# yjpark1/multiagent_rl

Measured on AMD Instinct MI355X. Metric: env-steps/sec, simple_spread N=6 x B envs, 1/2/4/8 MI355X, higher is better.
Workload: dtype f32

## Files before the change

multiagent_rl_amd/csrc/pw_kernels_spread_quad.hpp:

```cpp
#pragma once

#include "pw_kernels_spread.hpp"

namespace {

__device__ __forceinline__ void quad_pair_of(const int q, int &i, int &j)
{
    i = q < 5 ? 0 : q < 9 ? 1 : q < 12 ? 2 : q < 14 ? 3 : 4;
    j = q - (i == 0 ? 0 : i == 1 ? 5 : i == 2 ? 9 : i == 3 ? 12 : 14) + i + 1;
}

__device__ __forceinline__ void quad_act_fetch(const int32_t *row, const uint32_t lane_off, const uint32_t lds_slot, const uint32_t slot_read)
{
    unsigned keep;
    asm volatile("s_mov_b32 %0, m0\n\ts_mov_b32 m0, %3\n\ts_nop 0\n\tglobal_load_lds_dword %1, %2\n\ts_mov_b32 m0, %0"
                 : "=&s"(keep) : "v"(lane_off), "s"(row), "s"(lds_slot), "v"(slot_read) : "memory");
}

__device__ __forceinline__ float2 quad_action_force(const int ai, const float sens, const float fscale)
{
    float ux = 0.0f + ((ai == 1 ? 1.0f : 0.0f) - (ai == 2 ? 1.0f : 0.0f));
    float uy = 0.0f + ((ai == 3 ? 1.0f : 0.0f) - (ai == 4 ? 1.0f : 0.0f));
    ux *= sens; uy *= sens;
    if (fscale != 1.0f) { ux = fscale * ux; uy = fscale * uy; }
    return make_float2(ux + 0.0f, uy + 0.0f);
}

template <bool K1>
__device__ __forceinline__ void quad_pair_force(const float2 qi, const float2 qj, const uint32_t near_lo, const uint32_t near_span,
                                                const float dist_min, const float k, const float cf, float &Fx, float &Fy)
{
    const float dx = qi.x - qj.x, dy = qi.y - qj.y;
    const float d2 = dx * dx + dy * dy;
    const f32x2 a = {cf * dx, cf * dy};
    const bool near = __float_as_uint(d2) - near_lo >= near_span;
    const bool uni = (k >= 9.094947017729282e-13f) & (k <= 1099511627776.0f) & (cf >= 9.5367431640625e-07f) & (cf <= 128.0f);
    const bool c1 = (__float_as_uint(d2) - 0x12800000u) < (0x6C800000u - 0x12800000u);
    const bool c2 = fminf(fabsf(a.x), fabsf(a.y)) >= 8.673617379884035e-19f;
    const bool fast = near & c1 & c2 & uni;
    const bool any_cold = __builtin_amdgcn_ballot_w64(near & !fast) != 0;
    Fx = 0.0f; Fy = 0.0f;
    if (fast) {
        const float dist = sqrt_rn_core(d2);
        const float y0 = __builtin_amdgcn_rcpf(dist);
        __builtin_amdgcn_sched_barrier(0);
        const float yd = __builtin_fmaf(__builtin_fmaf(-dist, y0, 1.0f), y0, y0);
        const f32x2 Q = div_chain2(a, dist, yd);
        const float xarg = K1 ? div_chain1(-(dist - dist_min), k, div_refined_rcp(k))
                              : div_chain(-(dist - dist_min), k, div_refined_rcp(k));
        const float pen = softplus_branchless(xarg) * k;
        const f32x2 F = Q * f32x2{pen, pen};
        Fx = F.x;
        Fy = F.y;
    }
    if (__builtin_expect(any_cold, 0)) {
        if (near & !fast) collision_force_pair<true, K1>(qi.x, qi.y, qj.x, qj.y, dist_min, k, cf, Fx, Fy);
    }
}

template <bool COLL>
__device__ __forceinline__ void quad_coll_tests(const float2 mine, const float2 (&q6)[6], const float coll_thr2, int &cnt, uint32_t &cmask)
{
    cnt = 0; cmask = 0;
#if defined(PW_EXPERIMENTS) && defined(PW_EXP_NO_COLL_TESTS)
    cnt = 1;
#else
#pragma unroll
    for (int j = 0; j < 6; ++j) {
        const float2 q = q6[j];
        const float dx = q.x - mine.x, dy = q.y - mine.y;
        const float d2 = dx * dx + dy * dy;
        cnt += d2 < coll_thr2 ? 1 : 0;
        if (COLL) cmask |= d2 < coll_thr2 ? 1u << j : 0u;
    }
#endif
}

#ifndef PW_QUAD_BARRIER
#define PW_QUAD_BARRIER(t) duo_barrier()
#endif
#ifndef PW_QUAD_ACT_AHEAD
#define PW_QUAD_ACT_AHEAD 4
#endif
#ifndef PW_QUAD_PAD_P
#define PW_QUAD_PAD_P()
#endif
#ifndef PW_QUAD_PAD_OB
#define PW_QUAD_PAD_OB()
#endif
constexpr int kQuadActAhead = PW_QUAD_ACT_AHEAD;
constexpr int kQuadN = 6, kQuadL = 6, kQuadEPP = 4, kQuadEPW = 8;
struct SpreadQuadLds { float4 *s_ring; float2 *s_ftab, *s_lmB, *s_utab, *s_u; float *s_min, *s_rew; int32_t *s_act; uint32_t bytes; };
__host__ __device__ inline SpreadQuadLds spread_quad_lds(unsigned char *raw = nullptr)
{
    LdsCursor c{reinterpret_cast<float *>(raw)}; SpreadQuadLds o;
    o.s_ring = c.take<float4>(4 * kWave);
    o.s_ftab = c.take<float2>(2 * kQuadEPP * kQuadN * kQuadN);
    o.s_min = c.take<float>(kWave); o.s_rew = c.take<float>(kWave);
    o.s_lmB = c.take<float2>(kQuadEPW * kQuadL); o.s_act = c.take<int32_t>(2 * kQuadActAhead * kWave);
    o.s_u = reinterpret_cast<float2 *>(o.s_act + kQuadActAhead * kWave);
    o.s_utab = c.take<float2>(2 * 8);
    o.bytes = 4 * c.at; return o;
}
template <bool UNIT_MASS, bool COLL = false, bool K1 = false>
__global__ void __launch_bounds__(4 * kWave) pw_spread_quad_kernel(const StreamParams A, const int T)
{
    constexpr int N = kQuadN, L = kQuadL, D = 16, P2 = 15, EPP = kQuadEPP, EPW = kQuadEPW;
    extern __shared__ __attribute__((aligned(16))) unsigned char smem_raw[];
    const SpreadQuadLds Y = spread_quad_lds(smem_raw);

    const int wave = __builtin_amdgcn_readfirstlane((((int)threadIdx.x >> 6) + 2 * (((int)blockIdx.x >> 8) & 1)) & 3);
    const int lane = (int)threadIdx.x & 63;
    const int env0 = (int)blockIdx.x * EPW;
    const int envs_here = A.B - env0 < EPW ? A.B - env0 : EPW;
    const size_t BN = (size_t)A.B * N;

    const bool resets = A.auto_reset && A.max_episode_len > 0;
    int offs_all = A.ep_step[env0 + (lane < envs_here ? lane : 0)];
    auto next_reset_step = [&](int t_from) -> int {
        if (!resets) return 0x7fffffff;
        int rem = A.max_episode_len - 1 - (t_from + offs_all);
        rem = rem < 0 ? 0 : rem;
        int m = 0x7fffffff;
        for (int e = 0; e < envs_here; ++e) {
            const int r = __builtin_amdgcn_readlane(rem, e);
            m = r < m ? r : m;
        }
        return t_from + m;
    };
    int t_reset = next_reset_step(0);
    auto reset_step_update = [&](int t) {
        if (t + 1 + offs_all >= A.max_episode_len) offs_all = -(t + 1);
        t_reset = next_reset_step(t + 1);
    };
    int cur = 0;

    if (wave < 2) {
        __builtin_amdgcn_s_setprio(3);
        const int e0 = wave * EPP;
        const int nv = envs_here - e0 < 0 ? 0 : envs_here - e0 < EPP ? envs_here - e0 : EPP;
        if (nv == 0) {
            for (int t = 0; t < T; ++t) PW_QUAD_BARRIER(t);
            return;
        }
        const int la = lane < nv * N ? lane : 0;
        const int e4 = la / N, a = la - e4 * N;
        const int me = (e0 + e4) * N + a;
        const int env = env0 + e0 + e4;
        const uint32_t g = (uint32_t)env * (uint32_t)N + (uint32_t)a;
        const uint64_t env_id = A.env_id_base + (uint64_t)env;
        const int lp = lane < nv * P2 ? lane : 0;
        const int pe = lp / P2, pq = lp - pe * P2;
        int pi, pj;
        quad_pair_of(pq, pi, pj);
        const int ri = (e0 + pe) * N + pi, rj = (e0 + pe) * N + pj;
        float2 *ftab = Y.s_ftab + wave * (EPP * N * N);
        float2 *f_ij = ftab + (pe * N + pi) * N + (pj - 1), *f_ji = ftab + (pe * N + pj) * N + pi;
        const float2 *row = ftab + (e4 * N + a) * N;

        float px = A.pos_x[g], py = A.pos_y[g], vx = A.vel_x[g], vy = A.vel_y[g];
        int ep_off = A.ep_step[env];
        uint32_t ep_count = A.ep_count[env];
        Y.s_ring[me] = make_float4(px, py, vx, vy);
        float2 *u_w = Y.s_u + me;
        {
            const int32_t a0 = A.act[g], a1 = A.act[(T > 1 ? BN : (size_t)0) + g];
            u_w[0] = quad_action_force(a0, A.sens, A.fscale);
            u_w[kQuadEPW * N] = quad_action_force(a1, A.sens, A.fscale);
        }
        int u_at = 0;
        const float k = A.contact_margin, cf = A.contact_force, dt = A.dt, damp = A.damp, mass = A.mass;
        const uint32_t near_lo = __float_as_uint(A.near_thr2), near_span = 0x7F800000u - near_lo;
        float2 qi = *reinterpret_cast<const float2 *>(Y.s_ring + ri);
        float2 qj = *reinterpret_cast<const float2 *>(Y.s_ring + rj);
        PW_STAMP_DECL;
        for (int t = 0; t < T; ++t) {
            PW_STAMP_START;
            const float2 u0 = u_w[u_at];
            u_at = kQuadEPW * N - u_at;
            const bool two_slots = t == t_reset;
            float Fx, Fy;
            quad_pair_force<K1>(qi, qj, near_lo, near_span, A.dist_min, k, cf, Fx, Fy);
            *f_ij = make_float2(Fx, Fy);
            *f_ji = make_float2(-Fx, -Fy);
            PW_STAMP(0);
            float fx = u0.x, fy = u0.y;
            asm volatile("" ::: "memory");
#pragma unroll
            for (int j = 0; j < N - 1; ++j) {
                const float2 F = row[j];
                fx = F.x + fx;
                fy = F.y + fy;
            }
            vx = vx * damp; vy = vy * damp;
            vx = vx + div_mass<UNIT_MASS>(fx, mass) * dt;
            vy = vy + div_mass<UNIT_MASS>(fy, mass) * dt;
            px = px + vx * dt;
            py = py + vy * dt;
            int nxt = (cur + 1) & 3;
            Y.s_ring[nxt * kWave + me] = make_float4(px, py, vx, vy);
            if (__builtin_expect(two_slots, 0)) {
                if (t + 1 + ep_off >= A.max_episode_len) {
                    ep_count += 1;
                    ep_off = -(t + 1);
                    pw_reset_xy(A.seed, env_id, ep_count, (uint32_t)a, -1.0f, 1.0f, &px, &py);
                    vx = 0.f; vy = 0.f;
                }
                reset_step_update(t);
                nxt = (nxt + 1) & 3;
                Y.s_ring[nxt * kWave + me] = make_float4(px, py, vx, vy);
            }
            cur = nxt;
            asm volatile("" ::: "memory");
            qi = *reinterpret_cast<const float2 *>(Y.s_ring + cur * kWave + ri);
            qj = *reinterpret_cast<const float2 *>(Y.s_ring + cur * kWave + rj);
            PW_STAMP(1);
            PW_QUAD_PAD_P();
            PW_QUAD_BARRIER(t);
            PW_STAMP(2);
        }
#ifdef PW_STAMPS
        if (blockIdx.x == 0 && wave == 0 && lane == 0)
            for (int i_ = 0; i_ < 4; ++i_) g_pw_stamps[i_] = st_acc[i_];
#endif
        A.pos_x[g] = px; A.pos_y[g] = py;
        A.vel_x[g] = vx; A.vel_y[g] = vy;
        A.ep_step[env] = T + ep_off;
        A.ep_count[env] = ep_count;
        return;
    }

    int e_local = lane / N;
    int a = lane - e_local * N;
    if (e_local >= envs_here) { e_local = 0; a = 0; }
    const int env = env0 + e_local;
    const int base = e_local * N, me = base + a;
    const uint32_t g = (uint32_t)env * (uint32_t)N + (uint32_t)a;
    const uint64_t env_id = A.env_id_base + (uint64_t)env;
    int ep_off = A.ep_step[env];
    uint32_t ep_count = A.ep_count[env];
    float olx = A.lm_x[(size_t)env * L + a], oly = A.lm_y[(size_t)env * L + a];

    if (wave == 2) {
        float own_p = 0.0f;
        int cnt_p = 0;
        const int *cnt_w = reinterpret_cast<const int *>(Y.s_min) + lane;
        const int cnt_span = (int)(Y.s_rew - Y.s_min);
        int cnt_at = 0;
        int pre_last = 0;
        float2 q6[N];
        auto a_reads = [&](const int nxt) __attribute__((always_inline)) {
            const float4 *slot = Y.s_ring + nxt * kWave + base;
#pragma unroll
            for (int j = 0; j < N; ++j) q6[j] = *reinterpret_cast<const float2 *>(slot + j);
            pre_last = nxt;
        };
        float best, e0;
        auto a_dist = [&]() __attribute__((always_inline)) {
            float e2[N];
#pragma unroll
            for (int j = 0; j < N; ++j) {
                const float2 q = q6[j];
                const float ex = q.x - olx, ey = q.y - oly;
                e2[j] = ex * ex + ey * ey;
            }
            best = __builtin_fminf(__builtin_fminf(__builtin_fminf(e2[0], e2[1]), __builtin_fminf(e2[2], e2[3])),
                                   __builtin_fminf(e2[4], e2[5]));
            e0 = e2[0];
        };
        auto a_sqrt = [&]() __attribute__((always_inline)) -> float {
            const float b = e0 != e0 ? e0 : best;
            return sqrtf(b);
        };
        auto a_clock = [&](const int t, int nxt) __attribute__((always_inline)) {
            if (__builtin_expect(t == t_reset, 0)) {
                if (t + 1 + ep_off >= A.max_episode_len) {
                    ep_count += 1;
                    ep_off = -(t + 1);
                    pw_reset_xy(A.seed, env_id, ep_count, (uint32_t)(N + a), -1.0f, 1.0f, &olx, &oly);
                }
                reset_step_update(t);
                nxt = (nxt + 1) & 3;
            }
            cur = nxt;
        };
        float sh_own[L], sh_r[N], r;
        auto b_shfl_own = [&]() __attribute__((always_inline)) {
#pragma unroll
            for (int l = 0; l < L; ++l) sh_own[l] = __shfl(own_p, base + l, kWave);
        };
        auto b_reward = [&]() __attribute__((always_inline)) {
            r = 0.0f;
#pragma unroll
            for (int l = 0; l < L; ++l) r -= sh_own[l];
#pragma unroll
            for (int k2 = 0; k2 < N; ++k2) r -= k2 < cnt_p ? 1.0f : 0.0f;
#pragma unroll
            for (int i = 0; i < N; ++i) sh_r[i] = __shfl(r, base + i, kWave);
        };
        float *rew_t = A.rew, *rsh_t = A.rew_shared;
        auto b_store = [&]() __attribute__((always_inline)) {
            float acc = 0.0f;
#pragma unroll
            for (int i = 0; i < N; ++i) acc += sh_r[i];
            nt_store(rew_t + g, r);
            nt_store(rsh_t + env, acc);
            rew_t += BN; rsh_t += A.B;
        };
        PW_STAMP_DECL;
        {
            PW_STAMP_START;
            PW_QUAD_BARRIER(0);
            PW_STAMP(0);
            const int nxt = (cur + 1) & 3;
            a_reads(nxt);
            a_dist();
            own_p = a_sqrt();
            a_clock(0, nxt);
            PW_STAMP(1);
        }
        for (int t = 1; t < T; ++t) {
            PW_STAMP_START;
            PW_QUAD_BARRIER(t);
            PW_STAMP(0);
            const int nxt = (cur + 1) & 3;
            cnt_p = cnt_w[cnt_at];
            cnt_at = cnt_span - cnt_at;
            a_reads(nxt);
            b_shfl_own();
            a_dist();
            b_reward();
            const float own = a_sqrt();
            b_store();
            own_p = own;
            a_clock(t, nxt);
            PW_STAMP(1);
        }
        {
            const float4 *slot = Y.s_ring + pre_last * kWave + base;
            const float2 mine = *reinterpret_cast<const float2 *>(slot + a);
#pragma unroll
            for (int j = 0; j < N; ++j) q6[j] = *reinterpret_cast<const float2 *>(slot + j);
            uint32_t cmask;
            quad_coll_tests<false>(mine, q6, A.coll_thr2, cnt_p, cmask);
        }
        b_shfl_own();
        b_reward();
        b_store();
#ifdef PW_STAMPS
        if (blockIdx.x == 0 && lane == 0)
            for (int i_ = 0; i_ < 2; ++i_) g_pw_stamps[4 + i_] = st_acc[i_];
#endif
        return;
    }

    const int rows_here = envs_here * N;
    const int cgrp = lane & 3;
    const bool col0 = cgrp == 0;
    int row_u[3];
    uint32_t off_u[3];
#pragma unroll
    for (int u = 0; u < 3; ++u) {
        const int r = (lane >> 2) + 16 * u;
        const bool ok = r < rows_here;
        row_u[u] = ok ? r : 0;
        off_u[u] = (uint32_t)(ok ? lane + 64 * u : cgrp) * 16u;
    }
    float4 lm_u[3];
    auto load_landmarks = [&]() {
#pragma unroll
        for (int u = 0; u < 3; ++u)
            lm_u[u] = *reinterpret_cast<const float4 *>(Y.s_lmB + (row_u[u] / N) * L + (cgrp > 0 ? 2 * cgrp - 2 : 0));
    };
    Y.s_lmB[me] = make_float2(olx, oly);
    constexpr int kStepStores = 5 + (COLL ? 1 : 0);
    constexpr int kActBehind = kQuadActAhead * kStepStores + kQuadActAhead - 1;
    constexpr int kActWait = kActBehind < 63 ? kActBehind : 63;
    const unsigned char *act_row = reinterpret_cast<const unsigned char *>(A.act) + (size_t)(T > 2 ? 2 : T > 0 ? T - 1 : 0) * (BN * sizeof(int32_t));
    const size_t act_stride = BN * sizeof(int32_t);
    const uint32_t act_off = g * (uint32_t)sizeof(int32_t);
    const unsigned char *act_ring = reinterpret_cast<const unsigned char *>(Y.s_act + lane);
    uint32_t act_lds = __builtin_amdgcn_readfirstlane((uint32_t)reinterpret_cast<uintptr_t>(Y.s_act));
    asm volatile("" : "+s"(act_lds));
    constexpr uint32_t kSlotBytes = kWave * sizeof(int32_t), kRingMask = kQuadActAhead * kSlotBytes - 1;
    auto fetch_act = [&](int s, uint32_t slot_at, uint32_t slot_read) {
        quad_act_fetch(reinterpret_cast<const int32_t *>(act_row), act_off, act_lds + slot_at, slot_read);
        act_row += s + 1 < T ? act_stride : (size_t)0;
    };
    asm volatile("" :: "v"(ep_off), "v"(ep_count), "v"(offs_all), "v"(olx), "v"(oly), "s"(t_reset));
    for (int s0 = 2; s0 < 2 + kQuadActAhead; ++s0) fetch_act(s0, ((uint32_t)s0 * kSlotBytes) & kRingMask, 0u);
    if (lane < 6) Y.s_utab[lane] = quad_action_force(lane, A.sens, A.fscale);
    float2 *u_w = Y.s_u + me;
    int u_at = 0;
    uint32_t act_slot = (2 * kSlotBytes) & kRingMask;
    wave_lds_sync();
    load_landmarks();
    act_fetch_drain();
    unsigned char *obs_t = reinterpret_cast<unsigned char *>(A.obs + ((size_t)env0 * N) * D);
    uint8_t *done_t = A.done, *term_t = A.terminal;
    const size_t obs_stride = BN * D * sizeof(float);
    const bool has_len = A.max_episode_len > 0;
    int t_term = has_len ? A.max_episode_len - 1 - ep_off : 0x7fffffff;
    int *cnt_w = reinterpret_cast<int *>(Y.s_min) + lane;
    const int cnt_span = (int)(Y.s_rew - Y.s_min);
    int cnt_at = 0;
    uint64_t *coll_t = A.coll;
    PW_STAMP_DECL;
    for (int t = 0; t < T; ++t) {
        PW_STAMP_START;
        nt_store(done_t + g, (uint8_t)0);
        PW_QUAD_BARRIER(t);
        PW_STAMP(0);
        asm volatile("s_waitcnt vmcnt(%0)" :: "n"(kActWait) : "memory");
        const uint32_t ai = *reinterpret_cast<const uint32_t *>(act_ring + act_slot);
        int nxt = (cur + 1) & 3;
        float2 cmine, cq6[N];
        {
            const float4 *pre = Y.s_ring + nxt * kWave + base;
            cmine = *reinterpret_cast<const float2 *>(pre + a);
#pragma unroll
            for (int j = 0; j < N; ++j) cq6[j] = *reinterpret_cast<const float2 *>(pre + j);
        }
        fetch_act(t + 2 + kQuadActAhead, act_slot, ai);
        act_slot = (act_slot + kSlotBytes) & kRingMask;
        const float2 u2 = Y.s_utab[ai < 5u ? ai : 5u];
        nt_store(term_t + env, (uint8_t)(t >= t_term ? 1 : 0));
        if (t == t_reset) {
            const bool rst = t >= t_term;
            if (rst) {
                if (A.final_obs) {
                    const float4 st = Y.s_ring[nxt * kWave + me];
                    stream_write_obs<L>(A.final_obs + ((size_t)t * BN + g) * D, L, Y.s_lmB + base, st.x, st.y, st.z, st.w);
                }
                ep_count += 1;
                ep_off = -(t + 1);
                t_term = A.max_episode_len - 1 - ep_off;
                pw_reset_xy(A.seed, env_id, ep_count, (uint32_t)(N + a), -1.0f, 1.0f, &olx, &oly);
            }
            reset_step_update(t);
            wave_lds_sync();
            if (rst) Y.s_lmB[me] = make_float2(olx, oly);
            wave_lds_sync();
            load_landmarks();
            nxt = (nxt + 1) & 3;
        }
        cur = nxt;
        const float4 *slot = Y.s_ring + nxt * kWave;
        float4 st[3];
#pragma unroll
        for (int u = 0; u < 3; ++u) st[u] = slot[row_u[u]];
        {
            int cnt;
            uint32_t cmask;
            quad_coll_tests<COLL>(cmine, cq6, A.coll_thr2, cnt, cmask);
            cnt_w[cnt_at] = cnt;
            cnt_at = cnt_span - cnt_at;
            u_w[u_at] = u2;
            u_at = kQuadEPW * N - u_at;
            if (COLL) {
                nt_store(coll_t + g, (uint64_t)cmask);
                coll_t += BN;
            }
        }
        asm volatile("" :: "v"(st[0].x), "v"(st[0].y), "v"(st[0].z), "v"(st[0].w), "v"(st[1].x), "v"(st[1].y), "v"(st[1].z),
                           "v"(st[1].w), "v"(st[2].x), "v"(st[2].y), "v"(st[2].z), "v"(st[2].w));
#pragma unroll
        for (int u = 0; u < 3; ++u) {
            const float4 d = make_float4(lm_u[u].x - st[u].x, lm_u[u].y - st[u].y, lm_u[u].z - st[u].x, lm_u[u].w - st[u].y);
            const float4 o = make_float4(col0 ? st[u].z : d.x, col0 ? st[u].w : d.y, col0 ? st[u].x : d.z, col0 ? st[u].y : d.w);
            nt_store(reinterpret_cast<float4 *>(obs_t + off_u[u]), o);
        }
        obs_t += obs_stride; done_t += BN; term_t += A.B;
        PW_QUAD_PAD_OB();
        PW_STAMP(1);
    }
#ifdef PW_STAMPS
    if (blockIdx.x == 0 && lane == 0)
        for (int i_ = 0; i_ < 2; ++i_) g_pw_stamps[6 + i_] = st_acc[i_];
#endif
    A.lm_x[(size_t)env * L + a] = olx;
    A.lm_y[(size_t)env * L + a] = oly;
    act_fetch_drain();
}

}
```

multiagent_rl_amd/env.py:

```python
import ctypes as C

import numpy as np
import torch

from . import _lib
from ._lib import PwConfig, PwStateLayout, PwStepIO, check


class Discrete(object):

    def __init__(self, n):
        self.n = n
        self.shape = ()

    def sample(self):
        return int(np.random.randint(self.n))

    def __repr__(self):
        return 'Discrete(%d)' % self.n


class MultiDiscrete(object):

    def __init__(self, array_of_param_array):
        self.low = np.array([x[0] for x in array_of_param_array])
        self.high = np.array([x[1] for x in array_of_param_array])
        self.num_discrete_space = self.low.shape[0]
        self.shape = (self.num_discrete_space,)

    def sample(self):
        return [int(np.random.randint(lo, hi + 1)) for lo, hi in zip(self.low, self.high)]

    def __repr__(self):
        return 'MultiDiscrete' + str(self.num_discrete_space)


class Box(object):
    def __init__(self, shape, dtype=np.float32):
        self.shape = tuple(shape)
        self.dtype = dtype
        self.low, self.high_ = -np.inf, np.inf

    def __repr__(self):
        return 'Box%s' % (self.shape,)


def _ptr(t):
    return None if t is None else C.c_void_p(t.data_ptr())


def make_config(scenario_name, num_envs, num_agents=None, num_landmarks=None, num_adversaries=None,
                num_good=None, local_observation=True, max_episode_len=25, auto_reset=False,
                force_discrete_action=True, seed=12345678, env_id_base=0, action_force_uses_accel=False,
                **constants):
    lib = _lib.load()
    if scenario_name not in _lib.SCENARIOS:
        raise ValueError('unsupported scenario: %r (supported: %s)' % (scenario_name, sorted(_lib.SCENARIOS)))
    scen = _lib.SCENARIOS[scenario_name]
    if scen in (_lib.PW_SIMPLE_REFERENCE, _lib.PW_SIMPLE_SPEAKER_LISTENER):
        adv, n = 0, 2
    elif scen == _lib.PW_SIMPLE_TAG:
        adv = 3 if num_adversaries is None else int(num_adversaries)
        if num_good is None:
            num_good = 1 if num_agents is None else int(num_agents) - adv
        n = adv + int(num_good)
    else:
        adv = 0
        n = 3 if num_agents is None else int(num_agents)
    cfg = PwConfig()
    check(lib.pw_config_default(C.byref(cfg), scen, int(num_envs), n,
                                -1 if num_landmarks is None else int(num_landmarks), adv))
    cfg.obs_mode = _lib.PW_OBS_LOCAL if local_observation else _lib.PW_OBS_FULL
    cfg.max_episode_len = int(max_episode_len)
    cfg.auto_reset = int(bool(auto_reset))
    cfg.force_discrete_action = int(bool(force_discrete_action))
    cfg.action_force_uses_accel = int(bool(action_force_uses_accel))
    cfg.seed = int(seed) & 0xFFFFFFFFFFFFFFFF
    cfg.env_id_base = int(env_id_base)
    for k, v in constants.items():
        if k not in ('dt', 'damping', 'contact_force', 'contact_margin', 'default_sensitivity', 'mass',
                     'landmark_size'):
            raise TypeError('unknown world constant %r' % k)
        setattr(cfg, k, float(v))
    return cfg


class BatchedParticleEnv(object):

    def __init__(self, scenario_name='simple_spread', num_envs=1, device=None, config=None, want_coll=False,
                 dispatch=None, **kw):
        self.lib = _lib.load()
        if not torch.cuda.is_available():
            raise _lib.PworldError('BatchedParticleEnv needs a GPU: libpworld has no CPU fallback')
        self.device = torch.device('cuda', torch.cuda.current_device()) if device is None else torch.device(device)
        self.cfg = config if config is not None else make_config(scenario_name, num_envs, **kw)
        self.scenario_name = scenario_name
        h = C.c_void_p()
        check(self.lib.pw_create(C.byref(self.cfg), C.byref(h)))
        self._h = h
        if dispatch:
            self.set_dispatch(**dispatch)
        self.num_envs, self.n = self.cfg.num_envs, self.cfg.num_agents
        self.num_landmarks = self.cfg.num_landmarks
        self.obs_dim = self.lib.pw_obs_dim(h)
        self.want_coll = want_coll
        self.observation_space = [Box((self.obs_dim,)) for _ in range(self.n)]
        self.speaker_listener = self.cfg.scenario == _lib.PW_SIMPLE_SPEAKER_LISTENER
        self.dim_c = {_lib.PW_SIMPLE_REFERENCE: _lib.PW_DIM_C,
                      _lib.PW_SIMPLE_SPEAKER_LISTENER: _lib.PW_SL_DIM_C}.get(self.cfg.scenario, 0)
        if self.speaker_listener:
            if self.cfg.obs_mode != _lib.PW_OBS_LOCAL:
                raise NotImplementedError('simple_speaker_listener: only the observation the reference patches in '
                                          '(experiments/scenarios.py:45-64, local_observation=True) is built; '
                                          "upstream's has a different length per agent")
            self.action_space = [Discrete(self.dim_c), Discrete(5)]
            self.act_width = 5
        else:
            self.action_space = [MultiDiscrete([[0, 4], [0, self.dim_c - 1]]) if self.dim_c else Discrete(5)
                                 for _ in range(self.n)]
            self.act_width = 5 + self.dim_c
        with torch.cuda.device(self.device):
            self._state = torch.zeros(self.lib.pw_state_bytes(h), dtype=torch.uint8, device=self.device)
        check(self.lib.pw_bind_state(h, _ptr(self._state)))
        lay = PwStateLayout()
        check(self.lib.pw_get_state_layout(h, C.byref(lay)))
        self.layout = lay
        self.bytes_per_env_step = self.lib.pw_algorithmic_bytes_per_env_step(h)

    def __del__(self):
        h, self._h = getattr(self, '_h', None), None
        if h:
            self.lib.pw_destroy(h)

    def get_dispatch(self):
        d = _lib.PwDispatch()
        check(self.lib.pw_get_dispatch(self._h, C.byref(d)))
        return {n: int(getattr(d, n)) for n, _ in _lib.PwDispatch._fields_ if n != 'struct_size'}

    def set_dispatch(self, **fields):
        d = _lib.PwDispatch()
        check(self.lib.pw_get_dispatch(self._h, C.byref(d)))
        for k, v in fields.items():
            if k == 'struct_size' or not hasattr(d, k):
                raise TypeError('unknown pw_dispatch field %r' % k)
            setattr(d, k, int(v))
        check(self.lib.pw_set_dispatch(self._h, C.byref(d)))

    def set_actor_precision(self, mode):
        check(self.lib.pw_set_actor_precision(self._h, {'f32': 0, 'bf16x3': 1}[mode]))

    def get_actor_precision(self):
        return ('f32', 'bf16x3')[self.lib.pw_get_actor_precision(self._h)]

    def _stream(self):
        return C.c_void_p(torch.cuda.current_stream(self.device).cuda_stream)

    def _f32(self, *shape):
        return torch.empty(shape, dtype=torch.float32, device=self.device)

    def _dev(self, t, dtype):
        if t is None:
            return None
        t = torch.as_tensor(t)
        return t.to(device=self.device, dtype=dtype).contiguous()

    def set_state(self, pos, vel=None, landmarks=None, ep_step=None, ep_count=None, comm=None, goal=None):
        B, N, L = self.num_envs, self.n, self.num_landmarks
        if comm is not None or goal is not None:
            cm, gl = self._dev(comm, torch.float32), self._dev(goal, torch.int32)
            assert (cm is None or cm.shape == (B, N, self.dim_c)) and (gl is None or gl.shape == (B, N))
            check(self.lib.pw_set_comm_state(self._h, _ptr(cm), _ptr(gl), self._stream()))
        pos = self._dev(pos, torch.float32)
        vel = torch.zeros(B, N, 2, device=self.device) if vel is None else self._dev(vel, torch.float32)
        lm = self._dev(landmarks, torch.float32)
        assert pos.shape == (B, N, 2) and vel.shape == (B, N, 2) and (lm is None or lm.shape == (B, L, 2))
        es, ec = self._dev(ep_step, torch.int32), self._dev(ep_count, torch.int32)
        if (es is None) != (ec is None) or es is None:
            cur = self.get_state()
            es = cur['ep_step'] if es is None else es
            ec = cur['ep_count'] if ec is None else ec
        check(self.lib.pw_set_state(self._h, _ptr(pos), _ptr(vel), _ptr(lm), _ptr(es), _ptr(ec), self._stream()))

    def get_state(self):
        B, N, L = self.num_envs, self.n, self.num_landmarks
        out = dict(pos=self._f32(B, N, 2), vel=self._f32(B, N, 2), landmarks=self._f32(B, L, 2),
                   ep_step=torch.empty(B, dtype=torch.int32, device=self.device),
                   ep_count=torch.empty(B, dtype=torch.int32, device=self.device))
        check(self.lib.pw_get_state(self._h, _ptr(out['pos']), _ptr(out['vel']), _ptr(out['landmarks']),
                                    _ptr(out['ep_step']), _ptr(out['ep_count']), self._stream()))
        if self.dim_c:
            out['comm'] = self._f32(B, N, self.dim_c)
            out['goal'] = torch.empty(B, N, dtype=torch.int32, device=self.device)
            check(self.lib.pw_get_comm_state(self._h, _ptr(out['comm']), _ptr(out['goal']), self._stream()))
        return out

    def reset(self, mask=None):
        obs = self._f32(self.num_envs, self.n, self.obs_dim)
        m = self._dev(mask, torch.uint8)
        check(self.lib.pw_reset(self._h, _ptr(m), _ptr(obs), self._stream()))
        return obs

    def observe(self):
        obs = self._f32(self.num_envs, self.n, self.obs_dim)
        check(self.lib.pw_observe(self._h, _ptr(obs), self._stream()))
        return obs

    def reward(self):
        rew = self._f32(self.num_envs, self.n)
        if self.dim_c:
            coll = torch.zeros(self.num_envs, self.n, dtype=torch.int64, device=self.device)
            check(self.lib.pw_reward(self._h, _ptr(rew), None, self._stream()))
            return rew, coll
        coll = torch.empty(self.num_envs, self.n, dtype=torch.int64, device=self.device)
        check(self.lib.pw_reward(self._h, _ptr(rew), _ptr(coll), self._stream()))
        return rew, coll

    def alloc_outputs(self, T=None, coll=None, final_obs=True):
        B, N, D = self.num_envs, self.n, self.obs_dim
        lead = () if T is None else (T,)
        out = dict(obs=self._f32(*lead, B, N, D), rew=self._f32(*lead, B, N), rew_shared=self._f32(*lead, B),
                   done=torch.empty(*lead, B, N, dtype=torch.bool, device=self.device),
                   terminal=torch.empty(*lead, B, dtype=torch.bool, device=self.device))
        if final_obs and self.cfg.auto_reset:
            out['final_obs'] = self._f32(*lead, B, N, D)
        if self.want_coll if coll is None else coll:
            out['coll'] = torch.empty(*lead, B, N, dtype=torch.int64, device=self.device)
        return out

    def _io(self, actions, out, T):
        B, N = self.num_envs, self.n
        io = PwStepIO()
        lead = (B, N) if T is None else (T, B, N)
        actions = torch.as_tensor(actions)
        if actions.is_floating_point():
            a = actions.to(device=self.device, dtype=torch.float32).contiguous()
            assert a.shape == lead + (self.act_width,), 'float actions must be [..., B, N, %d]' % self.act_width
            io.act_vec = a.data_ptr()
        elif self.dim_c and not self.speaker_listener:
            assert actions.shape == lead + (2,), 'index actions must be [..., B, N, 2] (move, symbol)'
            a = actions.to(device=self.device, dtype=torch.int32)
            a = (a[..., 0].contiguous(), a[..., 1].contiguous())
            io.act_idx, io.act_comm = a[0].data_ptr(), a[1].data_ptr()
        else:
            a = actions.to(device=self.device, dtype=torch.int32).contiguous()
            assert a.shape == lead, 'index actions must be [..., B, N]'
            io.act_idx = a.data_ptr()
        for name in ('obs', 'final_obs', 'rew', 'rew_shared', 'done', 'terminal', 'coll'):
            t = out.get(name)
            if t is not None:
                assert t.is_contiguous() and t.device == self.device
                setattr(io, name, t.data_ptr())
        return io, a

    def plan_rollout(self, actions, out):
        T = int(actions.shape[0])
        io, keep = self._io(actions, out, T)
        fn, h, ref = self.lib.pw_rollout, self._h, C.byref(io)
        stream_of = self._stream

        def launch():
            rc = fn(h, ref, T, stream_of())
            if rc:
                check(rc)
        launch.keepalive = (io, keep, out)
        return launch

    def step(self, actions, out=None):
        out = self.alloc_outputs() if out is None else out
        io, keep = self._io(actions, out, None)
        check(self.lib.pw_step(self._h, C.byref(io), self._stream()))
        info = {k: out[k] for k in ('terminal', 'rew_shared', 'final_obs', 'coll') if k in out}
        return out['obs'], out['rew'], out['done'], info

    def last_kernel(self):
        return self.lib.pw_rollout_kernel(self._h).decode().strip('()').replace(', ', ',')

    def rollout(self, actions, out=None):
        T = int(actions.shape[0])
        out = self.alloc_outputs(T) if out is None else out
        io, keep = self._io(actions, out, T)
        check(self.lib.pw_rollout(self._h, C.byref(io), T, self._stream()))
        return out


class MultiAgentEnv(object):

    metadata = {'render.modes': ['human', 'rgb_array']}

    def __init__(self, scenario_name='simple_spread', n=None, local_observation=True, benchmark=False,
                 discrete_action=True, device=None, **kw):
        if scenario_name == 'simple_tag':
            kw.setdefault('num_agents', n)
        elif scenario_name == 'simple_spread':
            kw['num_agents'] = n
        self.batched = BatchedParticleEnv(scenario_name, 1, device=device, local_observation=local_observation,
                                          auto_reset=False, want_coll=benchmark, force_discrete_action=False,
                                          **kw)
        self.scenario_name = scenario_name
        self.n = self.batched.n
        cfg = self.batched.cfg
        self._A = cfg.num_adversaries if scenario_name == 'simple_tag' else 0
        self._L = cfg.num_landmarks
        D = self.batched.obs_dim
        if scenario_name == 'simple_tag':
            dims = [D if i < self._A or self._A == 0 else D - 2 for i in range(self.n)]
        else:
            dims = [D] * self.n
        self._dims = dims
        self.observation_space = [Box((d,)) for d in dims]
        self.action_space = list(self.batched.action_space)
        self._act_width = self.batched.act_width
        self.benchmark = benchmark
        self.discrete_action_space = discrete_action
        self.discrete_action_input = False
        self.force_discrete_action = False
        self.shared_reward = False
        self.time = 0
        self._reset_world()

    def seed(self, seed=None):
        return []

    def _reset_world(self):
        N, L = self.n, self._L
        goal = None
        if self.scenario_name == 'simple_reference':
            idx = list(range(L))
            goal = np.array([[np.random.choice(idx), np.random.choice(idx)]], dtype=np.int32)
        elif self.scenario_name == 'simple_speaker_listener':
            goal = np.array([[np.random.choice(list(range(L))), 0]], dtype=np.int32)
        lo = 0.9 if self.scenario_name == 'simple_tag' else 1.0
        pos = np.stack([np.random.uniform(-1, +1, 2) for _ in range(N)]) if N else np.zeros((0, 2))
        lm = np.stack([np.random.uniform(-lo, +lo, 2) for _ in range(L)]) if L else np.zeros((0, 2))
        z = torch.zeros(1, dtype=torch.int32)
        kw = {}
        if goal is not None:
            kw = dict(goal=torch.from_numpy(goal), comm=torch.zeros(1, N, self.batched.dim_c))
        self.batched.set_state(torch.from_numpy(pos[None].astype(np.float32)), None,
                               torch.from_numpy(lm[None].astype(np.float32)), ep_step=z, ep_count=z, **kw)

    def _rows(self, obs):
        obs = obs[0].cpu().numpy().astype(np.float64)
        return [obs[i, :d].copy() for i, d in enumerate(self._dims)]

    def reset(self):
        self._reset_world()
        return self._rows(self.batched.observe())

    def step(self, action_n):
        if self.scenario_name == 'simple_speaker_listener':
            a = np.zeros((1, self.n, self._act_width), np.float32)
            for i, x in enumerate(action_n):
                x = np.asarray(x, dtype=np.float32).reshape(self.action_space[i].n)
                a[0, i, :x.size] = x
        else:
            a = np.stack([np.asarray(x, dtype=np.float32).reshape(self._act_width) for x in action_n])[None]
        self._sync_force_discrete()
        obs, rew, done, info = self.batched.step(torch.from_numpy(a))
        rew_n = list(rew[0].cpu().numpy().astype(np.float64))
        done_n = [bool(x) for x in done[0].cpu().numpy()]
        if self.shared_reward:
            rew_n = [np.sum(rew_n)] * self.n
        info_n = {'n': [{} for _ in range(self.n)]}
        if self.benchmark:
            info_n = {'n': self._benchmark_data(rew_n, info['coll'][0].cpu().numpy())}
        return self._rows(obs), rew_n, done_n, info_n

    def _sync_force_discrete(self):
        want = int(bool(self.force_discrete_action))
        if getattr(self, '_fd_applied', None) != want:
            check(self.batched.lib.pw_set_force_discrete_action(self.batched._h, want))
            self._fd_applied = want

    def _benchmark_data(self, rew_n, coll):
        out = []
        if self.scenario_name == 'simple_tag':
            for i in range(self.n):
                c = int(coll[i]) & ((1 << self.n) - 1)
                out.append(bin(c >> self._A).count('1') if i < self._A else 0)
            return out
        st = self.batched.get_state()
        pos = st['pos'][0].cpu().numpy().astype(np.float64)
        lm = st['landmarks'][0].cpu().numpy().astype(np.float64)
        mins = [min(np.sqrt(np.sum(np.square(p - l))) for p in pos) for l in lm]
        min_dists = float(sum(mins))
        occupied = int(sum(1 for m in mins if m < 0.1))
        for i in range(self.n):
            c = int(coll[i]) & ((1 << self.n) - 1)
            out.append((rew_n[i], bin(c).count('1'), min_dists, occupied))
        return out

    def render(self, mode='human'):
        return []

    def close(self):
        pass
```

Measured before the change: 8.136 billion.

## Precompute episode-reset Philox draws ahead of time in observation wave

Moves the Philox random draws for agent and landmark resets out of the reset step. The observation wave now computes them ahead of the reset boundary, when all env clocks in the wave are aligned, and stashes the results in spare slots of the LDS state ring. Physics and landmark waves then read the precomputed positions instead of running pw_reset_xy on the critical path. This adds per-step Philox work during the draw window plus more bookkeeping for the reset schedule, and falls back to the old inline path when clocks differ.

```diff
diff --git a/multiagent_rl_amd/csrc/pw_kernels_spread_quad.hpp b/multiagent_rl_amd/csrc/pw_kernels_spread_quad.hpp
--- a/multiagent_rl_amd/csrc/pw_kernels_spread_quad.hpp
+++ b/multiagent_rl_amd/csrc/pw_kernels_spread_quad.hpp
@@ -88,13 +88,49 @@
 #ifndef PW_QUAD_PAD_OB
 #define PW_QUAD_PAD_OB()
 #endif
+#ifndef PW_QUAD_RESET_XY
+#define PW_QUAD_RESET_XY(kind, seed, env_id, episode, entity, x, y) pw_reset_xy(seed, env_id, episode, entity, -1.0f, 1.0f, x, y)
+#endif
+#ifndef PW_QUAD_DRAW_ROUNDS
+#define PW_QUAD_DRAW_ROUNDS 10
+#endif
+#ifndef PW_QUAD_DRAW_DELAY
+#define PW_QUAD_DRAW_DELAY 1
+#endif
 constexpr int kQuadActAhead = PW_QUAD_ACT_AHEAD;
 constexpr int kQuadN = 6, kQuadL = 6, kQuadEPP = 4, kQuadEPW = 8;
-struct SpreadQuadLds { float4 *s_ring; float2 *s_ftab, *s_lmB, *s_utab, *s_u; float *s_min, *s_rew; int32_t *s_act; uint32_t bytes; };
+constexpr int kQuadDrawRounds = PW_QUAD_DRAW_ROUNDS, kQuadDrawSlices = 10 / kQuadDrawRounds;
+constexpr int kQuadDrawDelay = PW_QUAD_DRAW_DELAY;
+constexpr int kQuadDrawDepth = kQuadDrawSlices + 1;
+static_assert(kQuadDrawRounds * kQuadDrawSlices == 10, "a slice is a whole number of Philox4x32-10's rounds");
+static_assert(kQuadDrawDelay >= 1, "the pipeline restarts behind the reset step");
+constexpr int kQuadNever = 0x7fffffff;
+__host__ __device__ inline bool quad_draw_engages(const int auto_reset, const int max_episode_len, const bool clocks_equal, const int steps_since_start)
+{
+    return auto_reset != 0 && max_episode_len > 0 && clocks_equal && steps_since_start >= kQuadDrawDepth;
+}
+__host__ __device__ inline int quad_draw_at(const int i) { return (i >> 5) * (2 * kWave) + (i & 31); }
+__host__ __device__ inline void quad_philox_round(uint32_t (&c)[4], const uint32_t k0, const uint32_t k1)
+{
+    const uint64_t p0 = (uint64_t)0xD2511F53u * c[0], p1 = (uint64_t)0xCD9E8D57u * c[2];
+    const uint32_t n0 = (uint32_t)(p1 >> 32) ^ c[1] ^ k0, n2 = (uint32_t)(p0 >> 32) ^ c[3] ^ k1;
+    c[1] = (uint32_t)p1; c[3] = (uint32_t)p0; c[0] = n0; c[2] = n2;
+}
+__host__ __device__ inline float2 quad_draw_xy(const uint32_t r0, const uint32_t r1)
+{
+    const float lo = -1.0f, hi = 1.0f;
+    const float span = hi - lo;
+    const float u0 = (float)(r0 >> 8) * 5.9604644775390625e-8f;
+    const float u1 = (float)(r1 >> 8) * 5.9604644775390625e-8f;
+    return make_float2(span * u0 + lo, span * u1 + lo);
+}
+struct SpreadQuadLds { float4 *s_ring; float2 *s_ftab, *s_lmB, *s_utab, *s_u, *s_drawA, *s_drawL; float *s_min, *s_rew; int32_t *s_act; uint32_t bytes; };
 __host__ __device__ inline SpreadQuadLds spread_quad_lds(unsigned char *raw = nullptr)
 {
     LdsCursor c{reinterpret_cast<float *>(raw)}; SpreadQuadLds o;
     o.s_ring = c.take<float4>(4 * kWave);
+    o.s_drawA = reinterpret_cast<float2 *>(o.s_ring + kQuadEPW * kQuadN);
+    o.s_drawL = reinterpret_cast<float2 *>(o.s_ring + 2 * kWave + kQuadEPW * kQuadN);
     o.s_ftab = c.take<float2>(2 * kQuadEPP * kQuadN * kQuadN);
     o.s_min = c.take<float>(kWave); o.s_rew = c.take<float>(kWave);
     o.s_lmB = c.take<float2>(kQuadEPW * kQuadL); o.s_act = c.take<int32_t>(2 * kQuadActAhead * kWave);
@@ -129,9 +165,18 @@
         return t_from + m;
     };
     int t_reset = next_reset_step(0);
+    auto clocks_equal = [&]() -> bool { return __builtin_amdgcn_ballot_w64(offs_all != __builtin_amdgcn_readfirstlane(offs_all)) == 0; };
+    int t_fast = quad_draw_engages(A.auto_reset, A.max_episode_len, clocks_equal(), t_reset) ? t_reset : -1;
     auto reset_step_update = [&](int t) {
-        if (t + 1 + offs_all >= A.max_episode_len) offs_all = -(t + 1);
-        t_reset = next_reset_step(t + 1);
+        if (t == t_fast) {
+            offs_all = -(t + 1);
+            t_reset = t + A.max_episode_len;
+            t_fast = quad_draw_engages(A.auto_reset, A.max_episode_len, true, A.max_episode_len - kQuadDrawDelay) ? t_reset : -1;
+        } else {
+            if (t + 1 + offs_all >= A.max_episode_len) offs_all = -(t + 1);
+            t_reset = next_reset_step(t + 1);
+            t_fast = quad_draw_engages(A.auto_reset, A.max_episode_len, clocks_equal(), t_reset - (t + kQuadDrawDelay)) ? t_reset : -1;
+        }
     };
     int cur = 0;
 
@@ -169,6 +214,7 @@
             u_w[kQuadEPW * N] = quad_action_force(a1, A.sens, A.fscale);
         }
         int u_at = 0;
+        const float2 *draw_r = Y.s_drawA + quad_draw_at(me);
         const float k = A.contact_margin, cf = A.contact_force, dt = A.dt, damp = A.damp, mass = A.mass;
         const uint32_t near_lo = __float_as_uint(A.near_thr2), near_span = 0x7F800000u - near_lo;
         float2 qi = *reinterpret_cast<const float2 *>(Y.s_ring + ri);
@@ -200,10 +246,16 @@
             int nxt = (cur + 1) & 3;
             Y.s_ring[nxt * kWave + me] = make_float4(px, py, vx, vy);
             if (__builtin_expect(two_slots, 0)) {
-                if (t + 1 + ep_off >= A.max_episode_len) {
+                const bool fast = t == t_fast;
+                if (fast || t + 1 + ep_off >= A.max_episode_len) {
                     ep_count += 1;
                     ep_off = -(t + 1);
-                    pw_reset_xy(A.seed, env_id, ep_count, (uint32_t)a, -1.0f, 1.0f, &px, &py);
+                    if (fast) {
+                        const float2 d = *draw_r;
+                        px = d.x; py = d.y;
+                    } else {
+                        PW_QUAD_RESET_XY(1, A.seed, env_id, ep_count, (uint32_t)a, &px, &py);
+                    }
                     vx = 0.f; vy = 0.f;
                 }
                 reset_step_update(t);
@@ -248,6 +300,7 @@
         const int cnt_span = (int)(Y.s_rew - Y.s_min);
         int cnt_at = 0;
         int pre_last = 0;
+        const float2 *draw_r = Y.s_drawL + quad_draw_at(me);
         float2 q6[N];
         auto a_reads = [&](const int nxt) __attribute__((always_inline)) {
             const float4 *slot = Y.s_ring + nxt * kWave + base;
@@ -274,10 +327,16 @@
         };
         auto a_clock = [&](const int t, int nxt) __attribute__((always_inline)) {
             if (__builtin_expect(t == t_reset, 0)) {
-                if (t + 1 + ep_off >= A.max_episode_len) {
+                const bool fast = t == t_fast;
+                if (fast || t + 1 + ep_off >= A.max_episode_len) {
                     ep_count += 1;
                     ep_off = -(t + 1);
-                    pw_reset_xy(A.seed, env_id, ep_count, (uint32_t)(N + a), -1.0f, 1.0f, &olx, &oly);
+                    if (fast) {
+                        const float2 d = *draw_r;
+                        olx = d.x; oly = d.y;
+                    } else {
+                        PW_QUAD_RESET_XY(2, A.seed, env_id, ep_count, (uint32_t)(N + a), &olx, &oly);
+                    }
                 }
                 reset_step_update(t);
                 nxt = (nxt + 1) & 3;
@@ -388,6 +447,20 @@
         act_row += s + 1 < T ? act_stride : (size_t)0;
     };
     asm volatile("" :: "v"(ep_off), "v"(ep_count), "v"(offs_all), "v"(olx), "v"(oly), "s"(t_reset));
+    uint32_t ca[4], cl[4];
+    float2 nlm = make_float2(0.0f, 0.0f);
+    const uint32_t seed_lo = (uint32_t)A.seed, seed_hi = (uint32_t)(A.seed >> 32);
+    float2 *draw_wa = Y.s_drawA + quad_draw_at(me), *draw_wl = Y.s_drawL + quad_draw_at(me);
+    int t_draw = kQuadNever;
+    auto draw_start = [&](int t_first) __attribute__((always_inline)) {
+        const bool go = t_fast >= 0;
+        t_draw = go ? t_first : kQuadNever;
+        ca[0] = (uint32_t)a; cl[0] = (uint32_t)(N + a);
+        ca[1] = cl[1] = ep_count + 1u;
+        ca[2] = cl[2] = (uint32_t)env_id;
+        ca[3] = cl[3] = (uint32_t)(env_id >> 32);
+    };
+    draw_start(0);
     for (int s0 = 2; s0 < 2 + kQuadActAhead; ++s0) fetch_act(s0, ((uint32_t)s0 * kSlotBytes) & kRingMask, 0u);
     if (lane < 6) Y.s_utab[lane] = quad_action_force(lane, A.sens, A.fscale);
     float2 *u_w = Y.s_u + me;
@@ -435,9 +508,11 @@
                 ep_count += 1;
                 ep_off = -(t + 1);
                 t_term = A.max_episode_len - 1 - ep_off;
-                pw_reset_xy(A.seed, env_id, ep_count, (uint32_t)(N + a), -1.0f, 1.0f, &olx, &oly);
+                if (t == t_fast) { olx = nlm.x; oly = nlm.y; }
+                else PW_QUAD_RESET_XY(4, A.seed, env_id, ep_count, (uint32_t)(N + a), &olx, &oly);
             }
             reset_step_update(t);
+            draw_start(t + kQuadDrawDelay);
             wave_lds_sync();
             if (rst) Y.s_lmB[me] = make_float2(olx, oly);
             wave_lds_sync();
@@ -471,6 +546,21 @@
             nt_store(reinterpret_cast<float4 *>(obs_t + off_u[u]), o);
         }
         obs_t += obs_stride; done_t += BN; term_t += A.B;
+        const int ph = t - t_draw;
+        if ((unsigned)ph < (unsigned)kQuadDrawSlices) {
+            uint32_t k0 = seed_lo + (uint32_t)(ph * kQuadDrawRounds) * 0x9E3779B9u, k1 = seed_hi + (uint32_t)(ph * kQuadDrawRounds) * 0xBB67AE85u;
+#pragma unroll
+            for (int r = 0; r < kQuadDrawRounds; ++r) {
+                quad_philox_round(ca, k0, k1);
+                quad_philox_round(cl, k0, k1);
+                k0 += 0x9E3779B9u; k1 += 0xBB67AE85u;
+            }
+            if (ph == kQuadDrawSlices - 1) {
+                nlm = quad_draw_xy(cl[0], cl[1]);
+                *draw_wa = quad_draw_xy(ca[0], ca[1]);
+                *draw_wl = nlm;
+            }
+        }
         PW_QUAD_PAD_OB();
         PW_STAMP(1);
     }
diff --git a/multiagent_rl_amd/env.py b/multiagent_rl_amd/env.py
--- a/multiagent_rl_amd/env.py
+++ b/multiagent_rl_amd/env.py
@@ -5,6 +5,8 @@
 
 from . import _lib
 from ._lib import PwConfig, PwStateLayout, PwStepIO, check
+
+QUAD_DRAW_DEPTH = 2
 
 
 class Discrete(object):
```

Measured after the change: 8.758 billion (median of 6 runs). 7.7% higher.
